# OpenGene/fastp

Measured on NVIDIA H100. Metric: pairs per second, 150 bp PE synthetic FASTQ (1 pair = 2 reads: reads_per_s = 2 x value), higher is better.
Workload: dtype u8

## Files before the change

### fastp_b200/csrc/fp_chain2.cuh

```cuda
#pragma once
#include "fp_device.cuh"

#ifndef FP_ITEM_UNROLL
#define FP_ITEM_UNROLL 1
#endif
#ifndef FP_DENSE_UNROLL
#define FP_DENSE_UNROLL 1
#endif
static constexpr int kItemUnroll = FP_ITEM_UNROLL, kDenseUnroll = FP_DENSE_UNROLL;

__device__ __forceinline__ void smem_inc(uint32_t addr) { asm volatile("red.shared.add.u32 [%0], 1;" :: "r"(addr) : "memory"); }
#define smem_inc_gt(addr, a, B) asm volatile("{ .reg .pred p; setp.gt.s32 p, %1, %2; @p red.shared.add.u32 [%0], 1; }" :: "r"(addr), "r"(a), "r"(B) : "memory")

struct TRead {
    uint32_t srow;
    uint32_t prow;
    int front, len;
    bool null, clean;
    __device__ __forceinline__ uint8_t* seq() const { return static_cast<uint8_t*>(__cvta_shared_to_generic(srow)); }
    __device__ __forceinline__ uint8_t* qual() const { return static_cast<uint8_t*>(__cvta_shared_to_generic(srow + (uint32_t)(c_p.tile * c_p.stride))); }
    __device__ __forceinline__ uint32_t* pl() const { return static_cast<uint32_t*>(__cvta_shared_to_generic(prow)); }
};
__device__ __forceinline__ TRead t_read(const uint8_t* seq, const uint32_t* pl, int len, bool clean) {
    TRead r; r.srow = smem_u32(seq); r.prow = smem_u32(pl); r.front = 0; r.len = len; r.null = false; r.clean = clean;
// ... 550 lines not shown
            const uint8_t b1 = s1[p1], b2 = s2[p2];
            if (b1 == (use_planes ? comp_clean(b2) : dev_complement(b2))) continue;
            if (role == 0) {
                const uint8_t nb = use_planes ? comp_clean(b1) : dev_complement(b1);
                if (r2.clean) t_patch_delta_clean(D, 1, r2.seq(), l2, r2.front + p2, b2, (uint8_t)q2, nb, (uint8_t)q1);
                else t_patch_delta(D, G, false, 1, r2.seq(), l2, r2.front + p2, b2, (uint8_t)q2, nb, (uint8_t)q1);
                s2[p2] = nb; q2p[p2] = (uint8_t)q1; g2s[p2] = nb; g2q[p2] = (uint8_t)q1;
                if (r2.clean) t_plane_set_base(pl2, PW, r2.front + p2, nb, (uint8_t)q1);
                corrected++;
                atomicAdd(&bc->fr[FP_FR_CORRECTION + (nb & 7) * 9], 1u);
                if (sink.count) {
                    const unsigned int slot = atomicAdd(sink.count, 1u);
                    if (slot < sink.cap) { fp_patch pt; pt.pair = pair_index; pt.pos = (uint16_t)(r2.front + p2); pt.which = 1; pt.base = nb; pt.qual = (uint8_t)q1; pt.old_base = b2; pt.old_qual = (uint8_t)q2; pt._pad = 0; sink.patches[slot] = pt; }
                }
            } else {
                const uint8_t nb = use_planes ? comp_clean(b2) : dev_complement(b2);
                if (r1.clean) t_patch_delta_clean(D, 0, r1.seq(), l1, r1.front + p1, b1, (uint8_t)q1, nb, (uint8_t)q2);
                else t_patch_delta(D, G, false, 0, r1.seq(), l1, r1.front + p1, b1, (uint8_t)q1, nb, (uint8_t)q2);
                s1[p1] = nb; q1p[p1] = (uint8_t)q2; g1s[p1] = nb; g1q[p1] = (uint8_t)q2;
                if (r1.clean) t_plane_set_base(pl1, PW, r1.front + p1, nb, (uint8_t)q2);
                corrected++;
                atomicAdd(&bc->fr[FP_FR_CORRECTION + (nb & 7) * 9], 1u);
                if (sink.count) {
                    const unsigned int slot = atomicAdd(sink.count, 1u);
                    if (slot < sink.cap) { fp_patch pt; pt.pair = pair_index; pt.pos = (uint16_t)(r1.front + p1); pt.which = 0; pt.base = nb; pt.qual = (uint8_t)q2; pt.old_base = b1; pt.old_qual = (uint8_t)q1; pt._pad = 0; sink.patches[slot] = pt; }
                }
            }
        }
    }
    return corrected;
}

#define FP_CORR_CAP 1024
__device__ __noinline__ bool t_correct_decide(const TRead r1, const TRead r2, int PW, const fp_ov_result ov, int row, int sub, int g,
                                              uint32_t* list, int* nlist, int cap, uint32_t* cm1, uint32_t* cm2) {
    FP_SMEM(r1.qual());    FP_SMEM(r2.qual());    FP_SMEM(r1.pl());    FP_SMEM(r2.pl());    FP_SMEM(list);    FP_SMEM(nlist);    FP_SMEM(cm1);    FP_SMEM(cm2);
    bool overflow = false;
    const int ol = ov.overlap_len;
    const int start1 = max(0, (int)ov.offset);
    const int start2 = r2.len - max(0, -(int)ov.offset) - 1;
    const uint8_t* q1p = r1.qual() + r1.front; const uint8_t* q2p = r2.qual() + r2.front;
    const signed char GOOD = 33 + 30, BAD = 33 + 14;
    const uint32_t *pl1 = r1.pl(), *pl2 = r2.pl();
    const int e = r2.front + r2.len - 1, jb = r2.len - 1 - start2;
    const unsigned gm = group_mask(g);
    const int nw = (ol + 31) >> 5;
    uint32_t mine[2] = {0u, 0u};
    #pragma unroll
    for (int kk = 0; kk < 2; kk++) {
        const int k = sub + g * kk;
        if (k < nw) {
            const int s0 = e - (jb + 32 * k) - 31, abit = r1.front + start1 + 32 * k;
            const uint32_t rn = __brev(tp_bits_z(pl2 + 2 * PW, s0));
            const uint32_t rl_ = __brev(tp_bits_z(pl2, s0)), rh = ~__brev(tp_bits_z(pl2 + PW, s0)) & ~rn;
            mine[kk] = ((tp_bits(pl1, abit) ^ rl_) | (tp_bits(pl1 + PW, abit) ^ rh) | (tp_bits(pl1 + 2 * PW, abit) ^ rn)) & low_mask(ol - 32 * k);
        }
    }
    #pragma unroll 1
    for (int k = 0; k < nw; k++) {
        const int kk = k / g;
        const uint32_t w = kk == 0 ? mine[0] : mine[1];
        uint32_t todo = __shfl_sync(gm, w, (lane_id() & ~(g - 1)) + (k % g));
        todo &= (g == 4 ? 0x11111111u : g == 2 ? 0x55555555u : 0xFFFFFFFFu) << sub;
        #pragma unroll 1
        while (todo) {
            const int i = 32 * k + __ffs(todo) - 1;
            todo &= todo - 1;
            const int p1 = start1 + i, p2 = start2 - i;
            const signed char q1 = (signed char)q1p[p1], q2 = (signed char)q2p[p2];
            int which;
            if (q1 >= GOOD && q2 <= BAD) which = 1;
            else if (q2 >= GOOD && q1 <= BAD) which = 0;
            else continue;
            const int P1 = r1.front + p1, P2 = r2.front + p2;
            const int slot = atomicAdd(nlist, 1);
            if (slot >= cap) { overflow = true; continue; }
            list[slot] = (uint32_t)row | ((uint32_t)which << 7) | ((uint32_t)(which ? P2 : P1) << 8) | ((uint32_t)(which ? P1 : P2) << 18);
            if (which) atomicOr(&cm2[P2 >> 5], 1u << (P2 & 31)); else atomicOr(&cm1[P1 >> 5], 1u << (P1 & 31));
        }
    }
    return overflow;
}

__device__ __noinline__ uint32_t t_correct_item(uint32_t entry, const uint8_t* tile0, int tile_array_bytes, int S, int T, const uint16_t* s_len, const uint32_t* cm,
                                            int CMW, const DeltaAcc D, BlockCounters* bc, const PatchSink sink, unsigned int pair_index) {
    FP_SMEM(tile0);    FP_SMEM(s_len);    FP_SMEM(cm);    FP_SMEM(D.cyc);    FP_SMEM(D.kmer);    FP_SMEM(D.qh);    FP_SMEM(bc);
    const int row = entry & 0x7F, which = (entry >> 7) & 1, P = (entry >> 8) & 0x3FF, Pp = (entry >> 18) & 0x3FF;
    const uint8_t* mseq = tile0 + (which * 2) * tile_array_bytes + row * S; const uint8_t* mqual = mseq + tile_array_bytes;
    const uint8_t* pseq = tile0 + ((which ^ 1) * 2) * tile_array_bytes + row * S; const uint8_t* pqual = pseq + tile_array_bytes;
    const uint32_t* mcm = cm + (which * T + row) * CMW;
    const int l0 = s_len[which * T + row], c = P + Pp;
    const uint8_t ob = mseq[P], oq = mqual[P], nb = comp_clean(pseq[Pp]), nq = pqual[Pp];
    const int side = which;
    atomicAdd(&D.qh[side * FP_QUAL_BINS + oq], -1);
    atomicAdd(&D.qh[side * FP_QUAL_BINS + nq], +1);
    if (P < D.cycles) {
        int* c0 = D.cyc + side * D.cycles * 20 + P * 20;
        int* co = c0 + ((0x43F21F0Fu >> (4 * (ob & 7))) & 0xF) * 4;
        int* cn = c0 + ((0x43F21F0Fu >> (4 * (nb & 7))) & 0xF) * 4;
        atomicAdd(&co[0], -1); atomicAdd(&cn[0], +1);
        if (oq >= '5') atomicAdd(&co[1], -1);
        if (nq >= '5') atomicAdd(&cn[1], +1);
        if (oq >= '?') atomicAdd(&co[2], -1);
        if (nq >= '?') atomicAdd(&cn[2], +1);
        atomicAdd(&co[3], 33 - (int)oq); atomicAdd(&cn[3], (int)nq - 33);
    }
    uint32_t Z = 0, V = 0, Zn = 0, Vn = 0, CMB = 0;
    #pragma unroll
    for (int k = 0; k < 9; k++) {
        const int pos = P - 4 + k;
        const bool inb = pos >= 0 && pos < l0;
        const uint32_t bb = inb ? mseq[pos] : (uint32_t)'N';
        const bool corr = inb && ((mcm[pos >> 5] >> (pos & 31)) & 1u);
        const int pp = c - pos;
        const uint32_t nn_ = corr ? (uint32_t)comp_clean(pseq[pp]) : bb;
        Z |= ((bb >> 1) & 3u) << (2 * k); V |= (bb != (uint32_t)'N' ? 1u : 0u) << k;
        Zn |= ((nn_ >> 1) & 3u) << (2 * k); Vn |= (nn_ != (uint32_t)'N' ? 1u : 0u) << k;
        CMB |= (corr ? 1u : 0u) << k;
    }
    int* km = D.kmer + side * FP_KMER_BINS;
    #pragma unroll
    for (int w = 0; w < 5; w++) {
        if ((CMB >> 5) & ((1u << w) - 1u)) continue;
        if (((V >> w) & 31u) == 31u) atomicAdd(&km[(Z >> (2 * w)) & 0x3FFu], -1);
        if (((Vn >> w) & 31u) == 31u) atomicAdd(&km[(Zn >> (2 * w)) & 0x3FFu], +1);
    }
    atomicAdd(&bc->fr[FP_FR_CORRECTION + (nb & 7) * 9], 1u);
    if (sink.count) {
        const unsigned int slot = atomicAdd(sink.count, 1u);
        if (slot < sink.cap) { fp_patch pt; pt.pair = pair_index; pt.pos = (uint16_t)P; pt.which = (uint8_t)which; pt.base = nb; pt.qual = nq; pt.old_base = ob; pt.old_qual = oq; pt._pad = 0; sink.patches[slot] = pt; }
    }
    return (uint32_t)ob | ((uint32_t)oq << 8) | ((uint32_t)nb << 16) | ((uint32_t)nq << 24);
}

__device__ __forceinline__ uint32_t t_correct_apply(uint32_t entry, uint8_t* tile0, int tile_array_bytes, int S, int T, uint32_t* planes, int PSTR, int PW,
                                                uint8_t* gseq, uint8_t* gqual) {
    const int row = entry & 0x7F, which = (entry >> 7) & 1, P = (entry >> 8) & 0x3FF, Pp = (entry >> 18) & 0x3FF;
    uint8_t* mseq = tile0 + (which * 2) * tile_array_bytes + row * S; uint8_t* mqual = mseq + tile_array_bytes;
    const uint8_t* pseq = tile0 + ((which ^ 1) * 2) * tile_array_bytes + row * S; const uint8_t* pqual = pseq + tile_array_bytes;
    const uint8_t nb = comp_clean(pseq[Pp]), nq = pqual[Pp];
    const uint32_t old = (uint32_t)mseq[P] | ((uint32_t)mqual[P] << 8);
    mseq[P] = nb; mqual[P] = nq; gseq[P] = nb; gqual[P] = nq;
    uint32_t* pl = planes + (which * T + row) * PSTR + (P >> 5);
    const uint32_t m = 1u << (P & 31);
    const int c2 = (nb >> 1) & 3; const bool n = (nb == 'N');
    if (!n && (c2 & 1)) atomicOr(&pl[0], m); else atomicAnd(&pl[0], ~m);
    if (!n && (c2 & 2)) atomicOr(&pl[PW], m); else atomicAnd(&pl[PW], ~m);
    if (n) atomicOr(&pl[2 * PW], m); else atomicAnd(&pl[2 * PW], ~m);
    if (nq < (uint8_t)c_p.qualified_qual) atomicOr(&pl[3 * PW], m); else atomicAnd(&pl[3 * PW], ~m);
    return old;
}

__device__ __forceinline__ int t_gap_scan(const uint8_t* ins, const uint8_t* norm, int cmax, int cmin) {
    if (cmax < cmin || cmax < 2) return -1;
    int p1 = 0, p2 = 0, runmin = 1 << 20, best = -1;
    for (int j = 0; j < cmax; j++) {
        const int c = j + 1;
        p1 += (ins[j] != norm[j]);
        const int p2n = p2 + (ins[j + 1] != norm[j]);
        if (c >= 2 && c >= cmin && runmin + p2n <= c / 8 - 1) best = c;
        runmin = min(runmin, p1 - p2n);
        p2 = p2n;
    }
    return best;
}

__device__ __noinline__ bool gap_may_hit(unsigned long long D1, unsigned long long D2, int cmax) {
    const int amax = cmax / 8 - 1;
    const int kmax = min(cmax, 64) >> 3;
    int S = 0, M = 0, c2 = 0;
    #pragma unroll 1
    for (int k = 1; k <= kmax; k++) {
        const uint32_t b1 = (uint32_t)D1 & 0xFFu, b2 = (uint32_t)D2 & 0xFFu;
        D1 >>= 8; D2 >>= 8;
        c2 += __popc(b2);
        #pragma unroll
        for (int i = 0; i < 8; i++) { S += (int)((b1 >> i) & 1u) - (int)((b2 >> i) & 1u); M = min(M, S); }
        const int v = c2 + M;
        if (v <= k - 1) return true;
        if (v > amax) return false;
    }
    return false;
}

__device__ __forceinline__ unsigned long long at_pack(int len, int pos, int bases) {
    return 1ull << 63 | (unsigned long long)(uint32_t)len | (unsigned long long)(uint16_t)(int16_t)pos << 32 | (unsigned long long)(uint32_t)bases << 48;
}
__device__ __forceinline__ int at_len(unsigned long long t) { return (int)(uint32_t)t; }
__device__ __forceinline__ int at_pos(unsigned long long t) { return (int)(int16_t)(uint16_t)(t >> 32); }
__device__ __forceinline__ int at_bases(unsigned long long t) { return (int)((t >> 48) & 0x7FFFu); }

__device__ __noinline__ unsigned long long t_trim_by_sequence(const TRead r, const uint8_t* adata, int alen, int matchReq, int aidx, int PW,
                                                              BlockCounters* bc, int sub, int g, const EventSink ev, unsigned int unit, int which) {
    FP_SMEM(r.seq());    FP_SMEM(r.pl());    FP_SMEM(bc);
    const int rlen = r.len;
    const uint8_t* rdata = r.seq() + r.front;
    if (alen < matchReq) return 0ull;
    int start = 0;
    if (alen >= 16) start = -4; else if (alen >= 12) start = -3; else if (alen >= 8) start = -2;
    bool found = false;
    int pos = 0;
    const bool planes = r.clean && c_p.adapter_clean[aidx];
    const bool planes64 = planes && alen <= 64;
    unsigned long long R_lo = 0, R_hi = 0, R_nn = 0, A_lo = 0, A_hi = 0, A_nn = 0;
    if (planes64) {
        const uint32_t* ap = c_p.adapter_planes + aidx * 24;
        A_lo = (unsigned long long)__ldg(ap) | ((unsigned long long)__ldg(ap + 1) << 32);
        A_hi = (unsigned long long)__ldg(ap + 8) | ((unsigned long long)__ldg(ap + 9) << 32);
        A_nn = (unsigned long long)__ldg(ap + 16) | ((unsigned long long)__ldg(ap + 17) << 32);
        const unsigned long long live = mask64(rlen);
        R_lo = tp_bits64(r.pl(), r.front) & live; R_hi = tp_bits64(r.pl() + PW, r.front) & live; R_nn = tp_bits64(r.pl() + 2 * PW, r.front) & live;
    }
    for (int p = start; p < 0 && p < rlen - matchReq && !found; p++) {
        const int cmplen = min(rlen - p, alen), so = -p, n = cmplen - so;
        int mm = 0;
        if (planes64) mm = __popcll(((R_lo ^ (A_lo >> so)) | (R_hi ^ (A_hi >> so)) | (R_nn ^ (A_nn >> so))) & mask64(n));
        else for (int k = 0; k < n; k++) mm += (adata[so + k] != rdata[k]);
        if (mm <= cmplen / 8) { found = true; pos = p; }
    }
    if (!found) {
        const int npos = rlen - matchReq;
        int my_p = 1 << 20;
        if (planes) {
            const uint32_t* alo = c_p.adapter_planes + aidx * 24; const uint32_t* ahi = alo + 8; const uint32_t* ann = alo + 16;
            const uint32_t *plo = r.pl(), *phi = r.pl() + PW, *pnn = r.pl() + 2 * PW;
            const int nw = (alen + 31) >> 5;
            auto full_check = [&](int p) -> bool {
                const int cmplen = min(rlen - p, alen);
                int mm = 0;
                for (int k = 0; k < nw && 32 * k < cmplen; k++) {
                    const int bit = r.front + p + 32 * k;
                    const uint32_t x = (tp_bits(plo, bit) ^ __ldg(alo + k)) | (tp_bits(phi, bit) ^ __ldg(ahi + k)) | (tp_bits(pnn, bit) ^ __ldg(ann + k));
                    mm += __popc(x & low_mask(cmplen - 32 * k));
// ... 506 lines not shown
    uint64_t* mbar = reinterpret_cast<uint64_t*>(smem + sl.off_mbar);
    uint8_t* tile_seq[2]; uint8_t* tile_qual[2];
    tile_seq[0] = smem + sl.off_tile;
    tile_qual[0] = tile_seq[0] + sl.tile_array_bytes;
    tile_seq[1] = tile_qual[0] + sl.tile_array_bytes;
    tile_qual[1] = tile_seq[1] + sl.tile_array_bytes;
    uint16_t* s_len = reinterpret_cast<uint16_t*>(smem + sl.off_len);
    uint8_t* s_clean = smem + sl.off_clean;
    unsigned int* s_kmer = reinterpret_cast<unsigned int*>(smem + sl.off_kmer);
    unsigned int* s_qhist = reinterpret_cast<unsigned int*>(smem + sl.off_qhist);
    BlockCounters* bc = reinterpret_cast<BlockCounters*>(smem + sl.off_bc);
    DeltaAcc D;
    D.cycles = S;
    D.cyc = reinterpret_cast<int*>(smem + sl.off_delta);
    D.kmer = reinterpret_cast<int*>(smem + sl.off_dkmer);
    D.qh = reinterpret_cast<int*>(smem + sl.off_dqh);
    uint32_t* s_rm = reinterpret_cast<uint32_t*>(smem + sl.off_rm);
    int* s_nrm = reinterpret_cast<int*>(s_rm + SIDES * (T + 4));
    const int NBK = (S + 31) >> 5;
    uint32_t* s_bk = s_rm + SIDES * (T + 4) + 4;
    int* s_nbk = reinterpret_cast<int*>(s_bk + SIDES * NBK * (T + 4));
    DeltaSinks sinks; sinks.rm = s_rm; sinks.nrm = s_nrm; sinks.T = T;
    int16_t* s_lut = reinterpret_cast<int16_t*>(smem + sl.off_lut);
    const int PW = sl.plane_words, PSTR = sl.plane_stride;
    uint32_t* tile_planes = reinterpret_cast<uint32_t*>(smem + sl.off_planes);
    DeltaReq* s_queue = reinterpret_cast<DeltaReq*>(smem + sl.off_queue);
    unsigned int* s_dummy = reinterpret_cast<unsigned int*>(smem + sl.off_dummy);
    int* s_qn = reinterpret_cast<int*>(smem + sl.off_next);
    sinks.q = s_queue; sinks.qn = &s_qn[0];
    uint32_t* s_corr = reinterpret_cast<uint32_t*>(smem + sl.off_corr);
    int* s_ncorr = reinterpret_cast<int*>(s_corr + FP_CORR_CAP);
    uint32_t* s_cm = reinterpret_cast<uint32_t*>(smem + sl.off_cm);
    const int CMW = sl.cm_words;

    if (((smem_u32(smem) + (uint32_t)sl.off_kmer) & 4095u) != 0u) __trap();
    for (int i = tid; i < SIDES * T * PSTR; i += kChainThreads) tile_planes[i] = 0;
    for (int i = tid; i < SIDES * FP_KMER_BINS; i += kChainThreads) s_kmer[i] = 0;
    for (int i = tid; i < SIDES * FP_QUAL_BINS * FP_QH_REP; i += kChainThreads) s_qhist[i] = 0;
    for (int i = tid; i < SIDES * S * 20; i += kChainThreads) D.cyc[i] = 0;
    for (int i = tid; i < SIDES * FP_KMER_BINS; i += kChainThreads) D.kmer[i] = 0;
    for (int i = tid; i < SIDES * FP_QUAL_BINS; i += kChainThreads) D.qh[i] = 0;
    for (int i = tid; i < (int)(sizeof(BlockCounters) / 4); i += kChainThreads) reinterpret_cast<unsigned int*>(bc)[i] = 0;
    for (int i = tid; i < S + 2; i += kChainThreads) { s_lut[i] = c_p.lut_ovlimit[i]; s_lut[(S + 2) + i] = c_p.lut_lowq[i]; s_lut[2 * (S + 2) + i] = c_p.lut_mindiff[i]; }
    if (tid == 0) { mbar_init(mbar, 1); s_qn[0] = 0; s_qn[1] = 0; s_qn[2] = 0; asm volatile("fence.mbarrier_init.release.cluster;" ::: "memory"); }

    const int HPR = S >> 1;
    const int ncols = SIDES * HPR;
    const int nsplit = sl.col_split;
    const bool col_active = tid < ncols * nsplit;
    const int my_part = tid / ncols, my_col = col_active ? tid % ncols : 0;
    const int my_side = my_col / HPR, my_hc = my_col % HPR;
    const int my_w = my_hc >> 1, my_half = my_hc & 1;
    ColAcc2 acc;
    #pragma unroll
    for (int c = 0; c < 2; c++)
        #pragma unroll
        for (int b = 0; b < NB; b++)
            #pragma unroll
            for (int k = 0; k < 4; k++) acc.v[c][b][k] = 0;

    constexpr int GL = PAIRED ? 4 : 2;
    constexpr int UPW = 32 / GL;
    const int sub = lane % GL;
    const bool lead = sub == 0;
    const unsigned gmask = group_mask(GL);
    const int glead = lane & ~(GL - 1);

    auto fill_lens = [&](long long t) {
        if (t >= a.n_tiles) return;
        const long long r0 = t * T;
        const int nr = (int)min((long long)T, a.b.n - r0);
        for (int i = tid; i < SIDES * T; i += kChainThreads) {
            const int sd = i / T, r = i % T;
            uint16_t ln = 0;
            if (r < nr) { ln = (sd == 0 ? a.b.len1 : a.b.len2)[r0 + r]; if (ln > S) ln = (uint16_t)S; }
            s_len[i] = ln;
            s_clean[i] = 1;
        }
    };
    fill_lens(blockIdx.x);
    __syncthreads();
    uint32_t parity = 0;
#ifdef FP_PHASE_TIMING
    long long tph[12] = {0, 0, 0, 0, 0, 0, 0, 0, 0, 0, 0, 0}, tlast = clock64();
#define FP_TP(k) do { const long long tn_ = clock64(); tph[k] += tn_ - tlast; tlast = tn_; } while (0)
#else
#define FP_TP(k) do { } while (0)
#endif

    #pragma unroll 1
    for (long long tix = blockIdx.x; tix < a.n_tiles; tix += gridDim.x) {
        const long long row0 = tix * T;
        const int rows = (int)min((long long)T, a.b.n - row0);
        if (tid == 0) {
            asm volatile("fence.proxy.async.shared::cta;" ::: "memory");
            const uint32_t bytes = (uint32_t)rows * (uint32_t)S;
            mbar_expect_tx(mbar, bytes * 2 * SIDES);
            tma_bulk_g2s(tile_seq[0], a.b.seq1 + row0 * S, bytes, mbar);
            tma_bulk_g2s(tile_qual[0], a.b.qual1 + row0 * S, bytes, mbar);
            if (PAIRED) {
                tma_bulk_g2s(tile_seq[1], a.b.seq2 + row0 * S, bytes, mbar);
                tma_bulk_g2s(tile_qual[1], a.b.qual2 + row0 * S, bytes, mbar);
            }
            s_qn[0] = 0; s_qn[1] = 0; s_qn[3] = 0;
            if (PAIRED && c_p.correction) *s_ncorr = 0;
        }
        mbar_wait(mbar, parity);
        FP_TP(0);
        parity ^= 1;
        for (int i = tid; i < SIDES * (T + 4) + 4 + SIDES * NBK * (T + 4) + SIDES * NBK; i += kChainThreads) s_rm[i] = 0;
        if (PAIRED && c_p.correction) for (int i = tid; i < SIDES * T * CMW; i += kChainThreads) s_cm[i] = 0;

        if (col_active)
            dense_tile(acc, tile_seq[my_side], tile_qual[my_side], s_len + my_side * T, rows, S, my_w * 4, my_half, 4 * my_part, 4 * nsplit, G, my_side);
        FP_TP(10);
        {
            const int nwords = (S + 31) >> 5;
            const uint32_t qq4 = (uint32_t)(c_p.qualified_qual & 0x7F) * 0x01010101u;
            const uint32_t cq4 = (uint32_t)(min(max(c_p.cr_q, 0), 127)) * 0x01010101u;
            const int total = SIDES * T * nwords;
            const bool want_cq = c_p.cut_right != 0;
            const bool word_major = ((S >> 2) & 15) != 0;
            const uint32_t it_div = word_major ? (uint32_t)(SIDES * T) : (uint32_t)nwords;
            const uint32_t it_magic = 0xFFFFFFFFu / it_div + 1u;
            #pragma unroll 1
            for (;;) {
                int base = 0;
                if (lane == 0) base = atomicAdd(&s_qn[2], 32);
                base = __shfl_sync(FULL_MASK, base, 0);
                if (base >= total) break;
                const int it = base + lane;
                if (it < total) {
                    const int qd = (int)__umulhi((uint32_t)it, it_magic), rd = it - qd * (int)it_div;
                    const int j = word_major ? qd : rd, rowi = word_major ? rd : qd;
                    const int sd = rowi >= T ? 1 : 0, rr2 = rowi - sd * T;
                    uint32_t lo = 0, hi = 0, nn = 0, lq = 0, cqw = 0;
                    if (rr2 < rows) {
                        const int n = (int)s_len[sd * T + rr2] - 32 * j;
                        if (n > 0) {
                            const uint8_t* tseq_sd = smem + sl.off_tile + sd * 2 * sl.tile_array_bytes; const uint8_t* tqual_sd = tseq_sd + sl.tile_array_bytes;
                            const uint8_t* sp = tseq_sd + rr2 * S + 32 * j; const uint8_t* qp = tqual_sd + rr2 * S + 32 * j;
                            uint8_t* qhb = smem + sl.off_qhist;
                            const uint32_t qsel = ((uint32_t)(lane & (FP_QH_REP - 1)) << 2) | ((uint32_t)sd * (FP_QUAL_BINS * FP_QH_REP * 4));
                            const uint32_t qaddr = smem_u32(qhb) + qsel;
                            uint32_t okm = 0, bad = 0, clo = 0, chi = 0;
                            #pragma unroll (kItemUnroll)
                            for (int k = 0; k < 4; k++) {
                                const uint2 sw = *reinterpret_cast<const uint2*>(sp + 8 * k), qw = *reinterpret_cast<const uint2*>(qp + 8 * k);
                                uint32_t f_lo, f_hi, f_nn, f_lq, f_ok, f_bad, f_cq;
                                plane_pair(sw.x, sw.y, qw.x, qw.y, qq4, f_lo, f_hi, f_nn, f_lq, f_ok, f_bad, cq4, f_cq, want_cq);
                                cqw = __byte_perm(cqw, f_cq, 0x7321);
                                lo = __byte_perm(lo, f_lo, 0x7321); hi = __byte_perm(hi, f_hi, 0x7321); nn = __byte_perm(nn, f_nn, 0x7321);
                                lq = __byte_perm(lq, f_lq, 0x7321); okm = __byte_perm(okm, f_ok, 0x7321); bad = __byte_perm(bad, f_bad, 0x7321);
                                const uint32_t cc = __byte_perm(code_mul4(sw.x), code_mul4(sw.y), 0x7310);
                                clo = __byte_perm(clo, chi, 0x5432); chi = __byte_perm(chi, cc, 0x7632);
                                const int rem = n - 8 * k;
                                if (!((qw.x | qw.y) & 0x80808080u)) {
                                    if (rem >= 8) {
                                        #pragma unroll
                                        for (int b8 = 0; b8 < 8; b8++) {
                                            const uint32_t w = b8 < 4 ? qw.x : qw.y;
                                            const int bb = b8 & 3;
                                            const uint32_t sh = bb == 0 ? (w << 4) : (w >> (8 * bb - 4));
                                            smem_inc(qaddr | (sh & 0xFF0u));
                                        }
                                    } else {
                                        #pragma unroll
// ... 76 lines not shown
                bool counted = false;
                if (active) {
                    tc_apply(r1, t_trim_and_cut(r1.seq(), r1.qual(), len0, c_p.trim_front1, c_p.trim_tail1, sub, GL, clean ? r1.pl() + 4 * PW : nullptr));
                    if (!r1.null && c_p.polyg && !t_polyg_cannot_trim(r1, PW, c_p.polyg_min)) { const int nl = r1.clean ? t_trim_polyg_planes(r1.pl(), PW, r1.front, r1.len, c_p.polyg_min) : t_trim_polyg(r1.seq() + r1.front, r1.len, c_p.polyg_min); if (nl != r1.len) { r1.len = nl; flags |= FP_F_POLYG_TRIMMED; } }
                    bool dimer = false;
                    if (!r1.null && c_p.adapter_enabled) {
                        bool trimmed = false;
                        if (c_p.has_r1) {
                            const unsigned long long t = t_trim_by_sequence(r1, c_p.adapters + c_p.adapter_r1_off, c_p.adapter_r1_len, 4, 0, PW, bc, sub, GL, a.events, (unsigned int)gi, 0);
                            if (t) { r1.len = at_len(t); apos = at_pos(t); abases += at_bases(t); trimmed = true; }
                        }
                        if (c_p.n_fasta > 0) trimmed |= t_trim_by_multi(r1, PW, apos, abases, bc, sub, GL, a.events, (unsigned int)gi, 0);
                        if (trimmed) { if (lead) atomicAdd(&bc->fr[FP_FR_ADAPTER_READS], 1u); flags |= FP_F_ADAPTER_TRIMMED; }
                        if (trimmed && r1.len <= c_p.dimer_max_len) dimer = true;
                    }
                    if (!r1.null && c_p.polyx) {
                        const uint32_t px = t_polyx_cannot_trim(r1, PW, c_p.polyx_min) ? 0u : t_trim_polyx(r1.seq() + r1.front, r1.len, c_p.polyx_min);
                        if (px) {
                            r1.len = px_len(px); pbase = px_base(px); plen = px_n(px);
                            if (lead) { atomicAdd(&bc->fr[FP_FR_POLYX_READS + pbase], 1u); atomicAdd(&bc->fr[FP_FR_POLYX_BASES + pbase], (unsigned)plen); }
                            flags |= FP_F_POLYX_TRIMMED;
                        }
                    }
                    if (!r1.null && c_p.max_len1 > 0 && c_p.max_len1 < r1.len) r1.len = c_p.max_len1;
                    result = t_pass_filter_pair(r1, PW, s_lut, sub, gmask);
                    if (dimer) { result = FP_FAIL_ADAPTER_DIMER; flags |= FP_F_ADAPTER_DIMER; }
                    const bool dupout = a.is_dup && a.is_dup[gi];
                    if (dupout) flags |= FP_F_DUPLICATE;
                    counted = !r1.null && result == FP_PASS_FILTER && !dupout;
                    if (lead) {
                        atomicAdd(&bc->fr[FP_FR_READSTATS + result], 1u);
                        if (counted) { post[0] += 1; post[1] += r1.len; }
                        a.out1[gi] = t_make_result(r1, result, result, flags, apos, abases, pbase, plen);
                    }
                }
                const bool keep_tail = counted && r1.front == 0;
                push_delta<SIDES>(sinks, active && lead, clean, 0, rr, 0, keep_tail ? r1.len : 0, len0, -1);
                push_delta<SIDES>(sinks, active && lead && counted && !keep_tail, clean, 0, rr, r1.front, r1.front, r1.front + r1.len, +1);
            } else {
                const int l1 = active ? s_len[rr] : 0, l2 = active ? s_len[T + rr] : 0;
                const bool clean1 = s_clean[rr] != 0, clean2 = s_clean[T + rr] != 0;
                warp_rl(0, active && lead ? 1u : 0u); warp_rl(1, active && lead ? (uint32_t)l1 : 0u);
                warp_rl(4, active && lead ? 1u : 0u); warp_rl(5, active && lead ? (uint32_t)l2 : 0u);
                TRead r1 = t_read(tile_seq[0] + rr * S, tile_planes + rr * PSTR, l1, clean1);
                TRead r2 = t_read(tile_seq[1] + rr * S, tile_planes + (T + rr) * PSTR, l2, clean2);
                int flags1 = 0, flags2 = 0, apos1 = 0, apos2 = 0, ab1 = 0, ab2 = 0, pb1 = 255, pb2 = 255, pl1n = 0, pl2n = 0;
                fp_ov_result ov; ov.overlapped = 0; ov.has_gap = 0; ov.offset = 0; ov.overlap_len = 0; ov.diff = 0;
                fp_ov_result ovA = ov;
                bool both = false, need_correct = false;
                if (active) {
                    tc_apply(r1, t_trim_and_cut(r1.seq(), r1.qual(), l1, c_p.trim_front1, c_p.trim_tail1, sub, GL, clean1 ? r1.pl() + 4 * PW : nullptr));
                    tc_apply(r2, t_trim_and_cut(r2.seq(), r2.qual(), l2, c_p.trim_front2, c_p.trim_tail2, sub, GL, clean2 ? r2.pl() + 4 * PW : nullptr));
                    both = !r1.null && !r2.null;
                    if (both && c_p.polyg) {
                        if (!t_polyg_cannot_trim(r1, PW, c_p.polyg_min)) { const int nl = r1.clean ? t_trim_polyg_planes(r1.pl(), PW, r1.front, r1.len, c_p.polyg_min) : t_trim_polyg(r1.seq() + r1.front, r1.len, c_p.polyg_min); if (nl != r1.len) { r1.len = nl; flags1 |= FP_F_POLYG_TRIMMED; } }
                        if (!t_polyg_cannot_trim(r2, PW, c_p.polyg_min)) { const int nl = r2.clean ? t_trim_polyg_planes(r2.pl(), PW, r2.front, r2.len, c_p.polyg_min) : t_trim_polyg(r2.seq() + r2.front, r2.len, c_p.polyg_min); if (nl != r2.len) { r2.len = nl; flags2 |= FP_F_POLYG_TRIMMED; } }
                    }
                    if (both && (c_p.adapter_enabled || c_p.correction || c_p.thread0)) {
                        ov = (clean1 && clean2) ? t_analyze_planes(r1, r2, PW, s_lut, sub, GL) : t_analyze_bytes(r1, r2, s_lut);
                        if (c_p.thread0 && lead) {
                            int isize = c_p.isize_max;
                            if (ov.overlapped) {
                                if (ov.offset > 0) isize = r1.len + r2.len - ov.overlap_len + r1.front + r2.front;
                                else isize = ov.overlap_len + r1.front + r2.front;
                            }
                            if (isize > c_p.isize_max) isize = c_p.isize_max;
                            if (c_p.isize_max < FP_MAX_ISIZE_SMEM) atomicAdd(&bc->isize[isize], 1u);
                            else red_add64(&G[L.off_isize + isize], 1ull);
                        }
                    }
                    if (both && c_p.allow_gap && (c_p.adapter_enabled || c_p.correction) && !ov.overlapped) ovA = t_analyze_gap(r1, r2, s_lut, sub, GL);
                    else ovA = ov;
                    need_correct = both && c_p.correction && !ovA.has_gap && ovA.overlapped && ovA.diff != 0;
                }
                bool corr_overflow = false;
                const bool distributed = need_correct && clean1 && clean2;
                if (PAIRED && c_p.correction) {
                    if (distributed)
                        corr_overflow = t_correct_decide(r1, r2, PW, ovA, rr, sub, GL, s_corr, s_ncorr, FP_CORR_CAP, s_cm + rr * CMW, s_cm + (T + rr) * CMW);
                    FP_TP(3);
                    __syncthreads();
                    FP_TP(4);
                    const int ncorr = min(*s_ncorr, FP_CORR_CAP);
                    for (int i = tid; i < ncorr; i += kChainThreads)
                        t_correct_item(s_corr[i], tile_seq[0], sl.tile_array_bytes, S, T, s_len, s_cm, CMW, D, bc, a.sink, (unsigned int)(row0 + (s_corr[i] & 0x7F)));
                    __syncthreads();
                    for (int i = tid; i < ncorr; i += kChainThreads) {
                        const uint32_t en = s_corr[i];
                        const int erow = en & 0x7F, ewhich = (en >> 7) & 1;
                        t_correct_apply(en, tile_seq[0], sl.tile_array_bytes, S, T, tile_planes, PSTR, PW,
                                        (ewhich ? a.b.seq2 : a.b.seq1) + (row0 + erow) * S, (ewhich ? a.b.qual2 : a.b.qual1) + (row0 + erow) * S);
                    }
                    __syncthreads();
                    FP_TP(5);
                    if (tid == 0) *s_ncorr = 0;
                }
                int res1 = FP_FAIL_LENGTH, res2 = FP_FAIL_LENGTH;
                bool counted = false;
                if (active) {
                    bool dimer = false;
                    if (need_correct) {
                        corr_overflow = (__ballot_sync(gmask, corr_overflow) != 0u);
                        int nc = 0;
                        if ((!distributed || corr_overflow) && sub < 2)
                            nc = t_correct(r1, r2, r1.pl(), r2.pl(), PW, ovA, a.b.seq1 + gi * S + r1.front, a.b.qual1 + gi * S + r1.front,
                                           a.b.seq2 + gi * S + r2.front, a.b.qual2 + gi * S + r2.front, (unsigned int)gi, a.sink, bc, D, G, l1, l2, sub);
                        __syncwarp(gmask);
                        int n2 = __shfl_sync(gmask, nc, glead), n1 = __shfl_sync(gmask, nc, glead + 1);
                        if (distributed) {
                            uint32_t any1 = 0, any2 = 0;
                            for (int k = 0; k < CMW; k++) { any1 |= s_cm[rr * CMW + k]; any2 |= s_cm[(T + rr) * CMW + k]; }
                            n1 += any1 ? 1 : 0; n2 += any2 ? 1 : 0;
                        }
                        if (n1 > 0) flags1 |= FP_F_CORRECTED;
                        if (n2 > 0) flags2 |= FP_F_CORRECTED;
                        if (lead && n1 + n2 > 0) atomicAdd(&bc->fr[FP_FR_CORRECTED_READS], (n1 > 0 && n2 > 0) ? 2u : 1u);
                    }
                    if (both && c_p.adapter_enabled) {
                        bool trimmed = false;
                        if (ovA.overlapped && ovA.offset < 0) {
                            const int ol = ovA.overlap_len;
                            const int nl1 = min(r1.len, ol + r2.front), nl2 = min(r2.len, ol + r1.front);
                            const int a1 = r1.len - nl1, a2 = r2.len - nl2;
                            if (lead) {
                                atomicAdd(&bc->fr[FP_FR_ADAPTER_BASES], (unsigned)(a1 + a2));
                                push_event(a.events, (unsigned int)gi, 0, FP_EV_PAIR, 0, r1.front + nl1, a1, 0);
                                push_event(a.events, (unsigned int)gi, 1, FP_EV_PAIR, 1, r2.front + nl2, a2, 0);
                            }
                            r1.len = nl1; r2.len = nl2;
                            ab1 += a1; ab2 += a2;
                            trimmed = true;
                        }
                        bool t1 = trimmed, t2 = trimmed;
                        if (!trimmed) {
                            if (c_p.has_r1) {
                                const unsigned long long t = t_trim_by_sequence(r1, c_p.adapters + c_p.adapter_r1_off, c_p.adapter_r1_len, 4, 0, PW, bc, sub, GL, a.events, (unsigned int)gi, 0);
                                t1 = t != 0ull;
                                if (t1) { r1.len = at_len(t); apos1 = at_pos(t); ab1 += at_bases(t); }
                            }
                            if (c_p.has_r2) {
                                const unsigned long long t = t_trim_by_sequence(r2, c_p.adapters + c_p.adapter_r2_off, c_p.adapter_r2_len, 4, 1, PW, bc, sub, GL, a.events, (unsigned int)gi, 1);
                                t2 = t != 0ull;
                                if (t2) { r2.len = at_len(t); apos2 = at_pos(t); ab2 += at_bases(t); }
                            }
                        }
                        if (c_p.n_fasta > 0) {
                            t1 |= t_trim_by_multi(r1, PW, apos1, ab1, bc, sub, GL, a.events, (unsigned int)gi, 0);
                            t2 |= t_trim_by_multi(r2, PW, apos2, ab2, bc, sub, GL, a.events, (unsigned int)gi, 1);
                        }
                        if (t1) { if (lead) atomicAdd(&bc->fr[FP_FR_ADAPTER_READS], 1u); flags1 |= FP_F_ADAPTER_TRIMMED; }
                        if (t2) { if (lead) atomicAdd(&bc->fr[FP_FR_ADAPTER_READS], 1u); flags2 |= FP_F_ADAPTER_TRIMMED; }
                        if ((t1 || t2) && r1.len <= c_p.dimer_max_len && r2.len <= c_p.dimer_max_len) dimer = true;
                    }
                    if (both && c_p.polyx) {
                        const uint32_t px1 = t_polyx_cannot_trim(r1, PW, c_p.polyx_min) ? 0u : t_trim_polyx(r1.seq() + r1.front, r1.len, c_p.polyx_min);
                        if (px1) {
                            r1.len = px_len(px1); pb1 = px_base(px1); pl1n = px_n(px1); flags1 |= FP_F_POLYX_TRIMMED;
                            if (lead) { atomicAdd(&bc->fr[FP_FR_POLYX_READS + pb1], 1u); atomicAdd(&bc->fr[FP_FR_POLYX_BASES + pb1], (unsigned)pl1n); }
                        }
                        const uint32_t px2 = t_polyx_cannot_trim(r2, PW, c_p.polyx_min) ? 0u : t_trim_polyx(r2.seq() + r2.front, r2.len, c_p.polyx_min);
                        if (px2) {
                            r2.len = px_len(px2); pb2 = px_base(px2); pl2n = px_n(px2); flags2 |= FP_F_POLYX_TRIMMED;
                            if (lead) { atomicAdd(&bc->fr[FP_FR_POLYX_READS + pb2], 1u); atomicAdd(&bc->fr[FP_FR_POLYX_BASES + pb2], (unsigned)pl2n); }
                        }
                    }
                    if (both) {
                        if (c_p.max_len1 > 0 && c_p.max_len1 < r1.len) r1.len = c_p.max_len1;
                        if (c_p.max_len2 > 0 && c_p.max_len2 < r2.len) r2.len = c_p.max_len2;
                    }
                    const bool dupout = a.is_dup && a.is_dup[gi];
                    if (dupout) { flags1 |= FP_F_DUPLICATE; flags2 |= FP_F_DUPLICATE; }
                    int pv = 0;
                    bool merge_done = false;
                    if (c_p.merge && both) {
                        ov = (clean1 && clean2) ? t_analyze_planes(r1, r2, PW, s_lut, sub, GL) : t_analyze_bytes(r1, r2, s_lut);
// ... 43 lines not shown
                        a.out2[gi] = t_make_result(r2, res2, pv, flags2, apos2, ab2, pb2, pl2n);
                        if (a.ov) a.ov[gi] = ov;
                    }
                }
                {
                    const bool removed = false;
                    const bool keep1 = counted && r1.front == 0 && !removed;
                    push_delta<SIDES>(sinks, active && lead && !removed, clean1, 0, rr, 0, keep1 ? r1.len : 0, l1, -1);
                    push_delta<SIDES>(sinks, active && lead && counted && !keep1, clean1, 0, rr, r1.front, r1.front, r1.front + r1.len, +1);
                    const bool keep2 = counted && r2.front == 0 && !removed;
                    push_delta<SIDES>(sinks, active && lead && !removed, clean2, 1, rr, 0, keep2 ? r2.len : 0, l2, -1);
                    push_delta<SIDES>(sinks, active && lead && counted && !keep2, clean2, 1, rr, r2.front, r2.front, r2.front + r2.len, +1);
                }
            }
            warp_rl(2, post[0]); warp_rl(3, post[1]);
            if (PAIRED) { warp_rl(6, post[2]); warp_rl(7, post[3]); }
        }

        FP_TP(6);
        __syncthreads();
        FP_TP(7);

        {
            if (col_active) {
                const int nr = s_nrm[my_side];
                if (nr > 0) dense_remove(s_bk + my_side * NBK * (T + 4), s_nbk + my_side * NBK, NBK, T + 4, my_part, nsplit, tile_seq[my_side], tile_qual[my_side], S, my_w * 4, my_half,
                                         D.cyc + my_side * S * 20, S);
            }
            FP_TP(11);
            {
                const int nwords = (S + 31) >> 5;
                const int nr0 = s_nrm[0], nr1 = SIDES > 1 ? s_nrm[SIDES - 1] : 0;
                const int total = (nr0 + nr1) * nwords;
                const uint32_t nw_magic = 0xFFFFFFFFu / (uint32_t)nwords + 1u;
                const uint32_t kdummy = smem_u32(s_dummy) + 4u * (uint32_t)lane;
                #pragma unroll 1
                for (;;) {
                    if (total == 0) break;
                    int base = 0;
                    if (lane == 0) base = atomicAdd(&s_qn[3], 32);
                    base = __shfl_sync(FULL_MASK, base, 0);
                    if (base >= total) break;
                    const int it = base + lane;
                    if (it < total) {
                        const int ei = (int)__umulhi((uint32_t)it, nw_magic), j = it - ei * nwords;
                        const int sd = ei >= nr0 ? 1 : 0;
                        const uint32_t e = s_rm[sd * (T + 4) + ei - sd * nr0];
                        const int row = e & 0xFF, lo = (e >> 8) & 0xFFF, hi = e >> 20;
                        const int a0 = max(lo - 32 * j, 0), b0 = min(hi - 32 * j, 32);
                        if (b0 > a0) {
                            const uint8_t* sp = smem + sl.off_tile + sd * 2 * sl.tile_array_bytes + row * S + 32 * j;
                            const uint32_t* pnn = tile_planes + (sd * T + row) * PSTR + 2 * PW;
                            hist_remove_chunk(sp, sp + sl.tile_array_bytes, j, low_mask(b0) & ~low_mask(a0), pnn[j], j > 0 ? pnn[j - 1] : 0u,
                                              smem_u32(D.qh) + (uint32_t)sd * (FP_QUAL_BINS * 4), smem_u32(D.kmer) + (uint32_t)sd * (FP_KMER_BINS * 4), kdummy);
                        }
                    }
                }
            }
            const int nreq = s_qn[0];
            #pragma unroll 1
            for (;;) {
                if (nreq == 0) break;
                int qi = 0;
                if (lane == 0) qi = atomicAdd(&s_qn[1], 1);
                qi = __shfl_sync(FULL_MASK, qi, 0);
                if (qi >= nreq) break;
                const DeltaReq rq = s_queue[qi];
                const int row = rq.a & 0xFF, side = (rq.a >> 8) & 1, sign = ((rq.a >> 10) & 1) ? -1 : +1;
                const int ctx0 = (int)(rq.a >> 12), rlo = (int)(rq.b & 0xFFFF), rhi = (int)(rq.b >> 16);
                const uint8_t* sq = smem + sl.off_tile + side * 2 * sl.tile_array_bytes + row * S; const uint8_t* ql = sq + sl.tile_array_bytes;
                if ((rq.a >> 9) & 1) dev_stat_positions_smem(D, side, sq, ql, ctx0, rlo, rhi, sign);
                else dev_stat_positions(G, side * 2 + 1, sq, ql, ctx0, rlo, rhi, sign);
            }
        }
        fill_lens(tix + gridDim.x);
        if (tid == 0) s_qn[2] = 0;
        FP_TP(8);
        __syncthreads();
        FP_TP(9);
    }

#ifdef FP_PHASE_TIMING
    if (blockIdx.x == 0 && lane == 0)
        printf("PHASE warp %2d col %d tma %lld colA %lld itemsA %lld totA %lld busyB1 %lld totB1 %lld corr %lld busyB2 %lld totB2 %lld colC %lld itemsC %lld totC %lld\n",
               warp, col_active ? 1 : 0, tph[0], tph[10], tph[1], tph[2], tph[3], tph[4], tph[5], tph[6], tph[7], tph[11], tph[8], tph[9]);
#endif
    __syncthreads();
    const int BIN_SLOT[NB] = {1, 3, 4, 6, 7};
    if (col_active) {
        #pragma unroll
        for (int c = 0; c < 2; c++) {
            const int cyc = my_hc * 2 + c;
            if (cyc >= L.cycles) continue;
            #pragma unroll
            for (int b = 0; b < NB; b++) {
                const unsigned int n = acc.v[c][b][0], n20 = acc.v[c][b][1], n30 = acc.v[c][b][2], sq = acc.v[c][b][3];
                if (n == 0) continue;
                const long long qs = (long long)sq - 33ll * (long long)n;
                #pragma unroll 1
                for (int pp = 0; pp < 2; pp++) {
                    const int st = my_side * 2 + pp;
                    if (n30) red_add64(&G[fp_off_cycle(&L, st, 0 * 8 + BIN_SLOT[b], cyc)], (unsigned long long)n30);
                    if (n20) red_add64(&G[fp_off_cycle(&L, st, 1 * 8 + BIN_SLOT[b], cyc)], (unsigned long long)n20);
                    red_add64(&G[fp_off_cycle(&L, st, 2 * 8 + BIN_SLOT[b], cyc)], (unsigned long long)n);
                    red_add64(&G[fp_off_cycle(&L, st, 3 * 8 + BIN_SLOT[b], cyc)], (unsigned long long)qs);
                }
            }
        }
    }
    #pragma unroll 1
    for (int i = tid; i < SIDES * FP_KMER_BINS; i += kChainThreads) {
        const unsigned int v = s_kmer[i];
        if (v) { const int sd = i / FP_KMER_BINS, k = kmer_ref_index(i % FP_KMER_BINS); red_add64(&G[fp_off_kmer(&L, sd * 2, k)], (unsigned long long)v); red_add64(&G[fp_off_kmer(&L, sd * 2 + 1, k)], (unsigned long long)v); }
    }
    #pragma unroll 1
    for (int i = tid; i < SIDES * FP_QUAL_BINS; i += kChainThreads) {
        unsigned int v = 0;
        #pragma unroll
        for (int c = 0; c < FP_QH_REP; c++) v += s_qhist[i * FP_QH_REP + c];
        if (v) { const int sd = i / FP_QUAL_BINS, k = i % FP_QUAL_BINS; red_add64(&G[fp_off_qualhist(&L, sd * 2, k)], (unsigned long long)v); red_add64(&G[fp_off_qualhist(&L, sd * 2 + 1, k)], (unsigned long long)v); }
    }
    #pragma unroll 1
    for (int i = tid; i < SIDES * S * 20; i += kChainThreads) {
        const int v = D.cyc[i];
        if (v == 0) continue;
        const int sd = i / (S * 20), rem = i % (S * 20), cyc = rem / 20, bin = (rem % 20) / 4, kind = rem & 3;
        if (cyc >= L.cycles) continue;
        const int gk = kind == 0 ? 2 : kind == 1 ? 1 : kind == 2 ? 0 : 3;
        red_add64(&G[fp_off_cycle(&L, sd * 2 + 1, gk * 8 + BIN_SLOT[bin], cyc)], (unsigned long long)(long long)v);
    }
    #pragma unroll 1
    for (int i = tid; i < SIDES * FP_KMER_BINS; i += kChainThreads) { const int v = D.kmer[i]; if (v) red_add64(&G[fp_off_kmer(&L, (i / FP_KMER_BINS) * 2 + 1, kmer_ref_index(i % FP_KMER_BINS))], (unsigned long long)(long long)v); }
    #pragma unroll 1
    for (int i = tid; i < SIDES * FP_QUAL_BINS; i += kChainThreads) { const int v = D.qh[i]; if (v) red_add64(&G[fp_off_qualhist(&L, (i / FP_QUAL_BINS) * 2 + 1, i % FP_QUAL_BINS)], (unsigned long long)(long long)v); }
    #pragma unroll 1
    for (int i = tid; i < FP_FR_WORDS; i += kChainThreads) { const unsigned int v = bc->fr[i]; if (v) red_add64(&G[L.off_filter + i], (unsigned long long)v); }
    if (c_p.isize_max < FP_MAX_ISIZE_SMEM) {
        #pragma unroll 1
        for (int i = tid; i <= c_p.isize_max; i += kChainThreads) { const unsigned int v = bc->isize[i]; if (v) red_add64(&G[L.off_isize + i], (unsigned long long)v); }
    }
    if (tid < 2 * L.n_stats && tid < 8) {
        const unsigned long long v = bc->rl[tid];
        if (v) red_add64(&G[(tid & 1) ? fp_off_length_sum(&L, tid >> 1) : fp_off_reads(&L, tid >> 1)], v);
    }
}
```

Baseline: 445.6 million.

## Rewrite correction items with bit-plane k-mer extraction and branchless shared reductions

The per-correction work now reads the 9-base neighbourhood from the 2-bit sequence planes and correction mask with funnel shifts and bit spreading, instead of nine byte loads with per-position branches. Conditional shared-memory atomics become unconditional red.shared adds with a zero operand, which removes divergence. The apply phase reuses the value computed in the item phase and updates the planes with XOR deltas. Patch-sink slots are reserved with one atomic per tile rather than one per item. The extra work is a few more shared reductions that add zero, more bit-manipulation logic, and a changed item-to-thread mapping.

```diff
diff --git a/fastp_b200/csrc/fp_chain2.cuh b/fastp_b200/csrc/fp_chain2.cuh
--- a/fastp_b200/csrc/fp_chain2.cuh
+++ b/fastp_b200/csrc/fp_chain2.cuh
@@ -656,73 +656,78 @@
     return overflow;
 }
 
-__device__ __noinline__ uint32_t t_correct_item(uint32_t entry, const uint8_t* tile0, int tile_array_bytes, int S, int T, const uint16_t* s_len, const uint32_t* cm,
-                                            int CMW, const DeltaAcc D, BlockCounters* bc, const PatchSink sink, unsigned int pair_index) {
-    FP_SMEM(tile0);    FP_SMEM(s_len);    FP_SMEM(cm);    FP_SMEM(D.cyc);    FP_SMEM(D.kmer);    FP_SMEM(D.qh);    FP_SMEM(bc);
+__device__ __forceinline__ void smem_add_if(uint32_t addr, int v, bool c) {
+    asm volatile("red.shared.add.s32 [%0], %1;" :: "r"(addr), "r"(c ? v : 0) : "memory");
+}
+
+__device__ __forceinline__ uint32_t t_bits9(const uint32_t* pl, int s, int nw) {
+    const int w = ((s + 32) >> 5) - 1;
+    const uint32_t lo = w >= 0 ? pl[w] : 0u, hi = w + 1 < nw ? pl[w + 1] : 0u;
+    return __funnelshift_r(lo, hi, (s + 32) & 31) & 0x1FFu;
+}
+
+__device__ __forceinline__ uint32_t spread9(uint32_t x) {
+    x = (x | (x << 8)) & 0x00FF00FFu; x = (x | (x << 4)) & 0x0F0F0F0Fu;
+    x = (x | (x << 2)) & 0x33333333u; return (x | (x << 1)) & 0x55555555u;
+}
+
+__device__ __forceinline__ uint32_t t_correct_item(uint32_t entry, const uint8_t* tile0, int tile_array_bytes, int S, int T, const uint16_t* s_len,
+                                                const uint32_t* planes, int PSTR, int PW, const uint32_t* cm, int CMW, const DeltaAcc D, BlockCounters* bc) {
+    FP_SMEM(tile0);    FP_SMEM(s_len);    FP_SMEM(planes);    FP_SMEM(cm);    FP_SMEM(D.cyc);    FP_SMEM(D.kmer);    FP_SMEM(D.qh);    FP_SMEM(bc);
     const int row = entry & 0x7F, which = (entry >> 7) & 1, P = (entry >> 8) & 0x3FF, Pp = (entry >> 18) & 0x3FF;
     const uint8_t* mseq = tile0 + (which * 2) * tile_array_bytes + row * S; const uint8_t* mqual = mseq + tile_array_bytes;
     const uint8_t* pseq = tile0 + ((which ^ 1) * 2) * tile_array_bytes + row * S; const uint8_t* pqual = pseq + tile_array_bytes;
-    const uint32_t* mcm = cm + (which * T + row) * CMW;
-    const int l0 = s_len[which * T + row], c = P + Pp;
+    const int l0 = s_len[which * T + row];
     const uint8_t ob = mseq[P], oq = mqual[P], nb = comp_clean(pseq[Pp]), nq = pqual[Pp];
     const int side = which;
     atomicAdd(&D.qh[side * FP_QUAL_BINS + oq], -1);
     atomicAdd(&D.qh[side * FP_QUAL_BINS + nq], +1);
-    if (P < D.cycles) {
-        int* c0 = D.cyc + side * D.cycles * 20 + P * 20;
-        int* co = c0 + ((0x43F21F0Fu >> (4 * (ob & 7))) & 0xF) * 4;
-        int* cn = c0 + ((0x43F21F0Fu >> (4 * (nb & 7))) & 0xF) * 4;
-        atomicAdd(&co[0], -1); atomicAdd(&cn[0], +1);
-        if (oq >= '5') atomicAdd(&co[1], -1);
-        if (nq >= '5') atomicAdd(&cn[1], +1);
-        if (oq >= '?') atomicAdd(&co[2], -1);
-        if (nq >= '?') atomicAdd(&cn[2], +1);
-        atomicAdd(&co[3], 33 - (int)oq); atomicAdd(&cn[3], (int)nq - 33);
-    }
-    uint32_t Z = 0, V = 0, Zn = 0, Vn = 0, CMB = 0;
-    #pragma unroll
-    for (int k = 0; k < 9; k++) {
-        const int pos = P - 4 + k;
-        const bool inb = pos >= 0 && pos < l0;
-        const uint32_t bb = inb ? mseq[pos] : (uint32_t)'N';
-        const bool corr = inb && ((mcm[pos >> 5] >> (pos & 31)) & 1u);
-        const int pp = c - pos;
-        const uint32_t nn_ = corr ? (uint32_t)comp_clean(pseq[pp]) : bb;
-        Z |= ((bb >> 1) & 3u) << (2 * k); V |= (bb != (uint32_t)'N' ? 1u : 0u) << k;
-        Zn |= ((nn_ >> 1) & 3u) << (2 * k); Vn |= (nn_ != (uint32_t)'N' ? 1u : 0u) << k;
-        CMB |= (corr ? 1u : 0u) << k;
-    }
-    int* km = D.kmer + side * FP_KMER_BINS;
+    {
+        const bool cy = P < D.cycles;
+        const uint32_t c0 = smem_u32(D.cyc + side * D.cycles * 20 + (cy ? P : 0) * 20);
+        const uint32_t co = c0 + ((0x43F21F0Fu >> (4 * (ob & 7))) & 0xF) * 16;
+        const uint32_t cn = c0 + ((0x43F21F0Fu >> (4 * (nb & 7))) & 0xF) * 16;
+        smem_add_if(co, -1, cy); smem_add_if(cn, +1, cy);
+        smem_add_if(co + 4, -1, cy && oq >= '5'); smem_add_if(cn + 4, +1, cy && nq >= '5');
+        smem_add_if(co + 8, -1, cy && oq >= '?'); smem_add_if(cn + 8, +1, cy && nq >= '?');
+        smem_add_if(co + 12, 33 - (int)oq, cy); smem_add_if(cn + 12, (int)nq - 33, cy);
+    }
+    const uint32_t* mpl = planes + (which * T + row) * PSTR;
+    const uint32_t* ppl = planes + ((which ^ 1) * T + row) * PSTR;
+    const uint32_t inb = low_mask(min(9, l0 - P + 4)) & ~low_mask(max(0, 4 - P));
+    const uint32_t lo = t_bits9(mpl, P - 4, PW), hi = t_bits9(mpl + PW, P - 4, PW), nn = t_bits9(mpl + 2 * PW, P - 4, PW);
+    const uint32_t CMB = t_bits9(cm + (which * T + row) * CMW, P - 4, CMW) & inb;
+    const uint32_t plo = __brev(t_bits9(ppl, Pp - 4, PW)) >> 23, phi = __brev(t_bits9(ppl + PW, Pp - 4, PW)) >> 23;
+    const uint32_t pnn = __brev(t_bits9(ppl + 2 * PW, Pp - 4, PW)) >> 23;
+    const uint32_t V = ~nn & inb, Vn = ~((nn & ~CMB) | (pnn & CMB)) & inb;
+    const uint32_t Z = spread9(lo) | (spread9(hi) << 1);
+    const uint32_t Zn = spread9((lo & ~CMB) | (plo & CMB)) | (spread9((hi & ~CMB) | (~phi & CMB)) << 1);
+    const uint32_t km = smem_u32(D.kmer + side * FP_KMER_BINS);
     #pragma unroll
     for (int w = 0; w < 5; w++) {
-        if ((CMB >> 5) & ((1u << w) - 1u)) continue;
-        if (((V >> w) & 31u) == 31u) atomicAdd(&km[(Z >> (2 * w)) & 0x3FFu], -1);
-        if (((Vn >> w) & 31u) == 31u) atomicAdd(&km[(Zn >> (2 * w)) & 0x3FFu], +1);
+        const bool own = ((CMB >> 5) & ((1u << w) - 1u)) == 0u;
+        smem_add_if(km + 4 * ((Z >> (2 * w)) & 0x3FFu), -1, own && ((V >> w) & 31u) == 31u);
+        smem_add_if(km + 4 * ((Zn >> (2 * w)) & 0x3FFu), +1, own && ((Vn >> w) & 31u) == 31u);
     }
     atomicAdd(&bc->fr[FP_FR_CORRECTION + (nb & 7) * 9], 1u);
-    if (sink.count) {
-        const unsigned int slot = atomicAdd(sink.count, 1u);
-        if (slot < sink.cap) { fp_patch pt; pt.pair = pair_index; pt.pos = (uint16_t)P; pt.which = (uint8_t)which; pt.base = nb; pt.qual = nq; pt.old_base = ob; pt.old_qual = oq; pt._pad = 0; sink.patches[slot] = pt; }
-    }
     return (uint32_t)ob | ((uint32_t)oq << 8) | ((uint32_t)nb << 16) | ((uint32_t)nq << 24);
 }
 
-__device__ __forceinline__ uint32_t t_correct_apply(uint32_t entry, uint8_t* tile0, int tile_array_bytes, int S, int T, uint32_t* planes, int PSTR, int PW,
-                                                uint8_t* gseq, uint8_t* gqual) {
-    const int row = entry & 0x7F, which = (entry >> 7) & 1, P = (entry >> 8) & 0x3FF, Pp = (entry >> 18) & 0x3FF;
+__device__ __forceinline__ void t_correct_apply(uint32_t entry, uint32_t v, uint8_t* tile0, int tile_array_bytes, int S, int T, uint32_t* planes, int PSTR,
+                                                int PW, uint8_t* gseq, uint8_t* gqual) {
+    const int row = entry & 0x7F, which = (entry >> 7) & 1, P = (entry >> 8) & 0x3FF;
     uint8_t* mseq = tile0 + (which * 2) * tile_array_bytes + row * S; uint8_t* mqual = mseq + tile_array_bytes;
-    const uint8_t* pseq = tile0 + ((which ^ 1) * 2) * tile_array_bytes + row * S; const uint8_t* pqual = pseq + tile_array_bytes;
-    const uint8_t nb = comp_clean(pseq[Pp]), nq = pqual[Pp];
-    const uint32_t old = (uint32_t)mseq[P] | ((uint32_t)mqual[P] << 8);
+    const uint8_t nb = (uint8_t)(v >> 16), nq = (uint8_t)(v >> 24);
     mseq[P] = nb; mqual[P] = nq; gseq[P] = nb; gqual[P] = nq;
     uint32_t* pl = planes + (which * T + row) * PSTR + (P >> 5);
-    const uint32_t m = 1u << (P & 31);
-    const int c2 = (nb >> 1) & 3; const bool n = (nb == 'N');
-    if (!n && (c2 & 1)) atomicOr(&pl[0], m); else atomicAnd(&pl[0], ~m);
-    if (!n && (c2 & 2)) atomicOr(&pl[PW], m); else atomicAnd(&pl[PW], ~m);
-    if (n) atomicOr(&pl[2 * PW], m); else atomicAnd(&pl[2 * PW], ~m);
-    if (nq < (uint8_t)c_p.qualified_qual) atomicOr(&pl[3 * PW], m); else atomicAnd(&pl[3 * PW], ~m);
-    return old;
+    const int sh = P & 31;
+    const uint32_t nbits = (nb == 'N' ? 4u : (uint32_t)((nb >> 1) & 3)) | (nq < (uint8_t)c_p.qualified_qual ? 8u : 0u);
+    const uint32_t obits = ((pl[0] >> sh) & 1u) | (((pl[PW] >> sh) & 1u) << 1) | (((pl[2 * PW] >> sh) & 1u) << 2) | (((pl[3 * PW] >> sh) & 1u) << 3);
+    const uint32_t d = nbits ^ obits;
+    atomicXor(&pl[0], (d & 1u) << sh);
+    atomicXor(&pl[PW], ((d >> 1) & 1u) << sh);
+    atomicXor(&pl[2 * PW], ((d >> 2) & 1u) << sh);
+    atomicXor(&pl[3 * PW], ((d >> 3) & 1u) << sh);
 }
 
 __device__ __forceinline__ int t_gap_scan(const uint8_t* ins, const uint8_t* norm, int cmax, int cmin) {
@@ -1395,7 +1400,8 @@
     __syncthreads();
     uint32_t parity = 0;
 #ifdef FP_PHASE_TIMING
-    long long tph[12] = {0, 0, 0, 0, 0, 0, 0, 0, 0, 0, 0, 0}, tlast = clock64();
+    long long tph[15] = {0, 0, 0, 0, 0, 0, 0, 0, 0, 0, 0, 0, 0, 0, 0}, tlast = clock64();
+    long long t_tiles = 0, t_ncorr = 0; int t_ncorr_max = 0;
 #define FP_TP(k) do { const long long tn_ = clock64(); tph[k] += tn_ - tlast; tlast = tn_; } while (0)
 #else
 #define FP_TP(k) do { } while (0)
@@ -1638,15 +1644,35 @@
                     __syncthreads();
                     FP_TP(4);
                     const int ncorr = min(*s_ncorr, FP_CORR_CAP);
-                    for (int i = tid; i < ncorr; i += kChainThreads)
-                        t_correct_item(s_corr[i], tile_seq[0], sl.tile_array_bytes, S, T, s_len, s_cm, CMW, D, bc, a.sink, (unsigned int)(row0 + (s_corr[i] & 0x7F)));
+#ifdef FP_PHASE_TIMING
+                    t_tiles++; t_ncorr += ncorr; t_ncorr_max = max(t_ncorr_max, ncorr);
+#endif
+                    if (tid == kChainThreads - 1 && a.sink.count && ncorr > 0) s_ncorr[1] = (int)atomicAdd(a.sink.count, (unsigned int)ncorr);
+                    static_assert(FP_CORR_CAP <= 2 * kChainThreads, "a thread keeps at most two items");
+                    const int mine = lane * (kChainThreads / 32) + warp;
+                    uint32_t item0 = 0, item1 = 0;
+                    #pragma unroll 1
+                    for (int i = mine; i < ncorr; i += kChainThreads) {
+                        const uint32_t v = t_correct_item(s_corr[i], tile_seq[0], sl.tile_array_bytes, S, T, s_len, tile_planes, PSTR, PW, s_cm, CMW, D, bc);
+                        if (i < kChainThreads) item0 = v; else item1 = v;
+                    }
+                    FP_TP(12);
                     __syncthreads();
-                    for (int i = tid; i < ncorr; i += kChainThreads) {
-                        const uint32_t en = s_corr[i];
+                    FP_TP(13);
+                    const unsigned int pbase = (unsigned int)s_ncorr[1];
+                    for (int i = mine; i < ncorr; i += kChainThreads) {
+                        const uint32_t en = s_corr[i], v = i < kChainThreads ? item0 : item1;
                         const int erow = en & 0x7F, ewhich = (en >> 7) & 1;
-                        t_correct_apply(en, tile_seq[0], sl.tile_array_bytes, S, T, tile_planes, PSTR, PW,
+                        t_correct_apply(en, v, tile_seq[0], sl.tile_array_bytes, S, T, tile_planes, PSTR, PW,
                                         (ewhich ? a.b.seq2 : a.b.seq1) + (row0 + erow) * S, (ewhich ? a.b.qual2 : a.b.qual1) + (row0 + erow) * S);
+                        const unsigned int slot = pbase + (unsigned int)i;
+                        if (a.sink.count && slot < a.sink.cap) {
+                            fp_patch pt; pt.pair = (unsigned int)(row0 + erow); pt.pos = (uint16_t)((en >> 8) & 0x3FF); pt.which = (uint8_t)ewhich;
+                            pt.base = (uint8_t)(v >> 16); pt.qual = (uint8_t)(v >> 24); pt.old_base = (uint8_t)v; pt.old_qual = (uint8_t)(v >> 8); pt._pad = 0;
+                            a.sink.patches[slot] = pt;
+                        }
                     }
+                    FP_TP(14);
                     __syncthreads();
                     FP_TP(5);
                     if (tid == 0) *s_ncorr = 0;
@@ -1856,8 +1882,10 @@
 
 #ifdef FP_PHASE_TIMING
     if (blockIdx.x == 0 && lane == 0)
-        printf("PHASE warp %2d col %d tma %lld colA %lld itemsA %lld totA %lld busyB1 %lld totB1 %lld corr %lld busyB2 %lld totB2 %lld colC %lld itemsC %lld totC %lld\n",
-               warp, col_active ? 1 : 0, tph[0], tph[10], tph[1], tph[2], tph[3], tph[4], tph[5], tph[6], tph[7], tph[11], tph[8], tph[9]);
+        printf("PHASE warp %2d col %d tma %lld colA %lld itemsA %lld totA %lld busyB1 %lld totB1 %lld corr %lld busyB2 %lld totB2 %lld colC %lld itemsC %lld totC %lld"
+               " cItems %lld cWait2 %lld cApply %lld cWait3 %lld tiles %lld ncorr %lld ncorrMax %d\n",
+               warp, col_active ? 1 : 0, tph[0], tph[10], tph[1], tph[2], tph[3], tph[4], tph[12] + tph[13] + tph[14] + tph[5], tph[6], tph[7],
+               tph[11], tph[8], tph[9], tph[12], tph[13], tph[14], tph[5], t_tiles, t_ncorr, t_ncorr_max);
 #endif
     __syncthreads();
     const int BIN_SLOT[NB] = {1, 3, 4, 6, 7};
```

New measurement: 451.1 million, median of 6. +1.3%, better.
